# MVME-HBUT/Faster-OreFSDet

Measured on AMD Instinct MI355X. Metric: images/sec at 640x640 25-shot (eval FPS: model(inputs) + device sync per image, bs=1 per GPU), higher is better.
Workload: dtype f32

## Files before the change

faster-orefsdet_amd/csrc/ore_common.h:

```cpp
#pragma once
#include <hip/hip_runtime.h>
#include <stdint.h>
#include <stdio.h>
#include "ore_hip.h"

void ore_set_error(const char* fmt, ...);
void ore_note_wino(int v);
int ore_last_wino(void);
void ore_note_launch(int code, int split);
void ore_flop_count_add(double flops);

#define ORE_CHECK_ARG(cond, ...)              \
    do {                                      \
        if (!(cond)) {                        \
            ore_set_error(__VA_ARGS__);       \
            return ORE_EINVAL;                \
        }                                     \
    } while (0)

#define ORE_HIP(call)                                                                   \
    do {                                                                                \
        hipError_t e_ = (call);                                                         \
        if (e_ != hipSuccess) {                                                         \
            ore_set_error("%s:%d %s -> %s", __FILE__, __LINE__, #call, hipGetErrorString(e_)); \
// ... 26 lines not shown
}

typedef __bf16 bf16x8_t __attribute__((ext_vector_type(8)));
__device__ __forceinline__ f32x4 from_bf16x4(s16x4 h) {
    const u32x2 u = __builtin_bit_cast(u32x2, h);
    return f32x4{__builtin_bit_cast(float, u.x << 16), __builtin_bit_cast(float, u.x & 0xffff0000u),
                 __builtin_bit_cast(float, u.y << 16), __builtin_bit_cast(float, u.y & 0xffff0000u)};
}
__device__ __forceinline__ float bf16_bits_to_f32(unsigned short h) { return __builtin_bit_cast(float, (unsigned)h << 16); }
struct ore_bf16_t { unsigned short v; };
__device__ __forceinline__ f32x4 ld4(const float* p) { return *reinterpret_cast<const f32x4*>(p); }
__device__ __forceinline__ f32x4 ld4(const ore_bf16_t* p) { return from_bf16x4(*reinterpret_cast<const s16x4*>(p)); }
__device__ __forceinline__ void st4(float* p, f32x4 v) { *reinterpret_cast<f32x4*>(p) = v; }
__device__ __forceinline__ void st4(ore_bf16_t* p, f32x4 v) { *reinterpret_cast<s16x4*>(p) = to_bf16x4(v); }
__device__ __forceinline__ float ld1(const float* p) { return *p; }
__device__ __forceinline__ float ld1(const ore_bf16_t* p) { return bf16_bits_to_f32(p->v); }

namespace oreroi {
int roi_predict_post(const float* h, int32_t C, int32_t h_parts, const float* h_bias, const float* cls_w, const float* cls_b,
                     const float* box_w, const float* box_b, const float* boxes, const int32_t* n_dev, int32_t n_host, int32_t cap,
                     const float* reg_weights4_host, float img_h, float img_w, float score_thresh, float nms_thresh,
                     int32_t topk, float* det_boxes, float* det_scores, int64_t* det_src, int32_t* det_count,
                     const float* post_dev, float* fin_boxes, float* fin_scores, int32_t* fin_count,
                     int32_t* host_count, void* workspace, size_t workspace_bytes, void* stream);
int roi_merge_classes(const float* det_boxes, const float* det_scores, const int32_t* det_count, int32_t K, int32_t cap,
                      const int64_t* class_ids, int32_t topk, const float* post_dev, float* fin_boxes, float* fin_scores,
                      int64_t* fin_classes, int32_t* fin_count, int32_t* host_count, void* stream);
struct PredictWs { size_t raw_boxes, c_boxes, raw_scores, c_scores, c_src, ok, keep, nms; };
inline PredictWs predict_ws_layout(int32_t cap) {
    const size_t c = (size_t)(cap > 0 ? cap : 1);
    PredictWs w{};
    size_t o = 256;
    w.raw_boxes = o; o += c * 16;
    w.c_boxes = o; o += c * 16;
    w.raw_scores = o; o += c * 4;
    w.c_scores = o; o += c * 4;
    w.c_src = o; o += c * 4;
    w.ok = o; o += c * 4;
    w.keep = o; o += c * 8;
    w.nms = (o + 255) & ~(size_t)255;
    return w;
}
}

namespace oremisc {
int correlation_classes(const float* q, int32_t q_ld, int32_t q_coff, int32_t n_levels, const int32_t* H, const int32_t* W, int32_t C,
                        int32_t K, const float* k11s, const float* k13s, const float* k31s, float* out, int32_t out_ld, void* stream);
// ... 3 lines not shown
```

faster-orefsdet_amd/csrc/ore_conv_internal.h:

```cpp
#pragma once
#include "ore_common.h"

namespace oreconv {

struct Lvl { int orow0, irow0, H, W, Ho, Wo; };

struct ConvP {
    const float* in; int in_ld, in_coff;
    int B, Cin;
    int nlev; Lvl lv[4];
    const float* w;
    int Cout, Cout16, kh, kw, stride, pad, M, K;
    const float* scale; const float* shift; int ep_stride; int relu_cout;
    const float* in_mul; const float* in_add; int in_relu;
    const float* add; int add_ld, add_coff, add_H, add_W;
    float* out; int out_ld, out_coff;
    float* colsum;
    int splitk, steps_per_split, nchunks;
    float* ws; int* tile_cnt;
    int bf16;
    int xmap;
    int sb;
    const float* wino;
    size_t w_lstride;
// ... 49 lines not shown
    X(64, 112, 4, 1) X(64, 128, 2, 2) X(64, 64, 2, 2) X(128, 64, 4, 1) X(128, 128, 2, 2) X(32, 128, 1, 4) X(128, 112, 4, 1) X(64, 80, 4, 1) X(32, 64, 2, 2)
#define ORE_KW_TILES(X) \
    X(16, 16) X(16, 32) X(16, 48) X(16, 64) X(16, 80) X(32, 16) X(32, 32) X(32, 48) X(32, 64) X(32, 80)
constexpr bool gs_fits(int bm, int bn, int ns) { return ((bm + bn) / 16 + 3) / 4 * (ns - 1) <= 63 && (size_t)ns * (bm + bn) * 64 <= 150 * 1024; }

struct ConvKnobs {
    int patch_mode = -1;
    int kw_mode = 1;
    int kw_force[4] = {};
    int gs_force[2] = {};
    int gs_ns = 3;
    int xmap_force = -1;
    int kw_nw_force = 0;
    int wino_mode = 1;
    int ws_sb_mode = 1;
    int ws_s2_mode = 1;
    int rf_mode = 1;
    int rf_force[3] = {};
    int kd_mode = 1;
    int kd_force[4] = {};
    int gd_mode = 1;
    int gd_force[3] = {};
    int gd_dbg = 0;
    int igemm[5] = {};
};
extern ConvKnobs g_knobs;

using ConvPlan = ore_conv_plan_t;
ConvPlan conv_plan(const ConvP& p, int req_splitk, size_t workspace_floats);
bool conv_wino_covers(int Cout, int Cin);
int wino_level_blocks(const ConvP& p, int gy, int* blk0);

int launch_ws(const ConvP& p, const ConvPlan& pl, hipStream_t st);
int launch_patch(const ConvP& p, const ConvPlan& pl, hipStream_t st);
int launch_igemm(const ConvP& p, const ConvPlan& pl, hipStream_t st);
int launch_wino(const ConvP& p, const ConvPlan& pl, hipStream_t st);
int launch_gd(const ConvP& p, const ConvPlan& pl, hipStream_t st);
int launch_kd(const ConvP& p, const ConvPlan& pl, hipStream_t st);
int launch_rf(const ConvP& p, const ConvPlan& pl, hipStream_t st);
int launch_gs(const ConvP& p, const ConvPlan& pl, hipStream_t st);
int launch_kw(const ConvP& p, const ConvPlan& pl, hipStream_t st);
int conv_gd_splitk(const float* in, int in_ld, const float* w, int M, int K, int Cout16, float* parts, int S, hipStream_t st);

}
```

faster-orefsdet_amd/csrc/ore_conv_plan.cpp:

```cpp
#include "ore_common.h"
#include "ore_conv_internal.h"

namespace oreconv {

ConvKnobs g_knobs;

namespace {

const ConvKnobs& K = g_knobs;

ConvPlan make_plan(int launcher, int bm, int bn, int b0, int b1, int b2, int b3, int gx, int gy, int xmap = 0, int splitk = 1, int sps = 0) {
    ConvPlan pl{};
    pl.launcher = launcher; pl.error = ORE_OK;
    pl.bm = bm; pl.bn = bn;
    pl.build[0] = b0; pl.build[1] = b1; pl.build[2] = b2; pl.build[3] = b3;
    pl.splitk = splitk; pl.steps_per_split = sps; pl.xmap = xmap;
    pl.gx = gx; pl.gy = gy;
    return pl;
}

ConvPlan none() { return ConvPlan{}; }

ConvPlan fail(int code) {
    ConvPlan pl{};
// ... 487 lines not shown
}

using namespace oreconv;

extern "C" int ore_conv_set_plan_override(int32_t BM, int32_t BN, int32_t WGM, int32_t WGN, int32_t WGK) {
    ConvKnobs& k = g_knobs;
    switch (BM) {
    case -1: k.patch_mode = BN; k.igemm[0] = 0; break;
    case -2: k.kw_mode = BN; k.igemm[0] = 0; break;
    case -3: k.kw_force[0] = BN; k.kw_force[1] = WGM; k.kw_force[2] = WGN; k.kw_force[3] = WGK; break;
    case -4: k.gs_force[0] = BN; k.gs_force[1] = WGM; if (WGN > 0) k.gs_ns = WGN; break;
    case -5: k.xmap_force = BN; break;
    case -6: k.kw_nw_force = BN; break;
    case -7: k.wino_mode = BN; break;
    case -8: k.ws_sb_mode = BN; break;
    case -9: k.ws_s2_mode = BN; break;
    case -10: k.rf_mode = BN; break;
    case -11: k.rf_force[0] = BN; k.rf_force[1] = WGM; k.rf_force[2] = WGN; break;
    case -12: k.kd_mode = BN; break;
    case -13: k.kd_force[0] = BN; k.kd_force[1] = WGM; k.kd_force[2] = WGN; k.kd_force[3] = WGK; break;
    case -14: k.gd_mode = BN; break;
    case -15: k.gd_force[0] = BN; k.gd_force[1] = WGM; k.gd_force[2] = WGN; break;
    case -16: k.gd_dbg = BN; break;
    default: k.igemm[0] = BM; k.igemm[1] = BN; k.igemm[2] = WGM; k.igemm[3] = WGN; k.igemm[4] = WGK; break;
    }
    return ORE_OK;
}

extern "C" int ore_conv_reset_plan_overrides(void) {
    g_knobs = ConvKnobs{};
    return ORE_OK;
}
```

faster-orefsdet_amd/csrc/ore_engine.hip:

```cpp
#include <map>
#include <string>
#include <vector>
#include <math.h>
#include <string.h>
#include "ore_common.h"
#include "ore_conv_internal.h"
#include <algorithm>


namespace {

struct HostTensor { std::vector<float> v; std::vector<int64_t> shape; };

struct Conv {
    float* w = nullptr; float* scale = nullptr; float* shift = nullptr;
    uint16_t* wh = nullptr;
    float* wino = nullptr;
    int Cin = 0, Cout = 0, k = 1, stride = 1, pad = 0, relu_cout = 0;
};

struct Buf { float* p = nullptr; int ld = 0; size_t rows = 0; };

struct Geo { int B, H, W, Hp, Wp; int h[6], w[6]; };

// ... 417 lines not shown
int run_detect_classes(ore_engine* e, const Geo& g, hipStream_t st, int K) {
    ore_detect_desc d[ORE_MAX_CLASSES];
    for (int k = 0; k < K; ++k) {
        d[k] = ore_detect_desc{};
        detect_desc(e, g, k, d[k]);
        if (k > 0) d[k].workspace = e->det_ws_slots + (size_t)(k - 1) * e->det_ws_bytes;
    }
    return ore_detect_batch_fwd(d, K, st);
}

int run_roi(ore_engine* e, const Geo& g, hipStream_t st, double* flops, int b = 0, bool class_slot = false) {
    const ore_model_cfg& c = e->cfg;
    float* roi_W = class_slot ? e->roi_W_slot[b] : e->roi_W;
    float* roi_b = class_slot ? e->roi_b_slot[b] : e->roi_b;
    const int F = c.fpn_ch;
    const size_t cap = (size_t)3 * c.pre_topk, rcap = (size_t)e->roi_cap;
    float* out_boxes = e->out_boxes + b * cap * 4;
    int32_t* counts = e->counts + b * 4;
    const float* feat[3]; int ld[3], coff[3], H[3], W[3]; float sc[3];
    for (int l = 0; l < 3; ++l) {
        feat[l] = e->at(e->pcat.p, ((size_t)lvl_row0(g, l) + (size_t)b * g.h[l + 3] * g.w[l + 3]) * 2 * F); ld[l] = 2 * F; coff[l] = F;
        H[l] = g.h[l + 3]; W[l] = g.w[l + 3]; sc[l] = 1.0f / (float)c.strides[l];
    }
    int rc = e->sb() ? ore_roi_align_bf16_fwd(reinterpret_cast<const uint16_t* const*>(feat), ld, coff, H, W, sc, 3, 3, F, e->roi_pooled, out_boxes,
                                              counts + 1, 0, e->roi_cap, e->roi_feat, st)
                     : ore_roi_align_fwd(feat, ld, coff, H, W, sc, 3, 3, F, e->roi_pooled, out_boxes, counts + 1, 0, e->roi_cap, e->roi_feat, st);
    if (rc) return rc;
    const int K = e->roi_pooled * e->roi_pooled * F;
    Run r{e, st};
    r.prof = e->profiling;
    Conv fc{};
    fc.w = roi_W; fc.scale = nullptr; fc.shift = roi_b; fc.Cin = K; fc.Cout = e->roi_fc; fc.k = 1; fc.stride = 1; fc.pad = 0;
    fc.relu_cout = e->roi_fc;
    const int S = e->roi_ksplit;
    if (S > 1) {
        const double fl = 2.0 * (double)e->roi_cap * K * e->roi_fc;
        hipEvent_t ea = nullptr, eb = nullptr;
        size_t ia = 0;
        if (r.prof) { ia = e->ev_used; ea = e->next_event(); eb = e->next_event(); if (ea) (void)hipEventRecord(ea, st); }
        rc = oreconv::conv_gd_splitk(e->roi_feat, K, roi_W, e->roi_cap, K, e->roi_fc, e->roi_hp, S, st);
        if (r.prof && ea && eb) { (void)hipEventRecord(eb, st); e->spans.push_back({ia, ia + 1, fl, fl}); }
        if (rc) return rc;
        *flops = fl;
    } else {
        PrecisionScope fp32(ORE_CONV_FP32);
        r.conv(fc, e->roi_feat, K, 0, 1, 1, e->roi_cap, e->roi_h, e->roi_fc, 0);
        if (r.rc) return r.rc;
        *flops = r.flops;
    }
    return oreroi::roi_predict_post(S > 1 ? e->roi_hp : e->roi_h, e->roi_fc, S > 1 ? S : 0, S > 1 ? roi_b : nullptr, e->roi_cls_w, e->roi_cls_b,
                                    e->roi_box_w, e->roi_box_b, out_boxes, counts + 1, 0,
                                    e->roi_cap, e->roi_reg_w, (float)g.H, (float)g.W, e->roi_score_thresh, e->roi_nms_thresh, e->roi_topk,
                                    e->det_boxes + b * rcap * 4, e->det_scores + b * rcap, e->det_src + b * rcap, e->det_count + b * 4,
                                    class_slot ? nullptr : e->post, e->fin_boxes_of(b), e->fin_scores_of(b), e->fin_count + b * 4,
                                    b == 0 && !class_slot ? e->pin_count_dev : nullptr, e->roi_ws, e->roi_ws_bytes, st);
}

}

extern "C" int ore_engine_set_roi_head(ore_engine* e, const float* W_host, const float* b_host, int32_t fc_dim, int32_t pooled,
                                       const float* cls_w_host, const float* cls_b_host, const float* box_w_host,
                                       const float* box_b_host, const float* reg_weights4_host, float score_thresh, float nms_thresh,
                                       int32_t topk) {
    ORE_CHECK_ARG(e && e->finalized && W_host && b_host && cls_w_host && cls_b_host && box_w_host && box_b_host && reg_weights4_host,
                  "ore_engine_set_roi_head: engine must be finalized, pointers non-null");
    ORE_CHECK_ARG(fc_dim % 16 == 0 && fc_dim > 0 && pooled >= 1 && pooled <= 16 && nms_thresh > 0.f, "ore_engine_set_roi_head: bad args");
    ORE_CHECK_ARG((size_t)fc_dim * 4 * 71 + 6 * 64 * 4 <= 60 * 1024,
                  "ore_engine_set_roi_head: fc width %d: the fused second-stage kernels cover fc widths up to 208 (FC_DIM/8 = 128 in finetune_vovnet.yaml)", fc_dim);
    static_assert(ORE_DET_RECORD_ROWS <= 512, "k_roi_tail<1024> sorts at most 512 candidates");
    ORE_HIP(hipSetDevice(e->device));
    const size_t K = (size_t)pooled * pooled * e->cfg.fpn_ch;
    int rc;
    auto up = [&](float** dst, const float* src, size_t n) -> int {
        if (!*dst && (rc = e->dalloc(dst, n))) return rc;
        ORE_HIP(hipMemcpy(*dst, src, n * sizeof(float), hipMemcpyHostToDevice));
        return ORE_OK;
    };
    if (e->roi_set && (e->roi_fc != fc_dim || e->roi_pooled != pooled)) { ore_set_error("ore_engine_set_roi_head: shape change not supported"); return ORE_EINVAL; }
// ... 629 lines not shown
```

faster-orefsdet_amd/csrc/ore_roi.hip:

```cpp
#include "ore_common.h"
#include <stdlib.h>

#ifdef ORE_TRACE
__device__ unsigned long long* g_trace_roi = nullptr;
#define ROI_TR(i) do { if (g_trace_roi && threadIdx.x == 0) g_trace_roi[(i)] = __builtin_amdgcn_s_memtime(); } while (0)
extern "C" int ore_debug_set_trace_roi(unsigned long long* buf) {
    return hipMemcpyToSymbol(HIP_SYMBOL(g_trace_roi), &buf, sizeof(buf)) == hipSuccess ? 0 : -5;
}
#else
#define ROI_TR(i) do { } while (0)
#endif

namespace {

__device__ __forceinline__ float ore_expf(float x) {
    if (x > 88.0f) x = 88.0f;
    if (x < -87.0f) x = -87.0f;
    const float n = rintf(x * 1.44269504088896341f);
    float r = fmaf(n, -0.693359375f, x);
    r = fmaf(n, 2.12194440e-4f, r);
    float p = 1.9875691500e-4f;
    p = fmaf(p, r, 1.3981999507e-3f);
    p = fmaf(p, r, 8.3334519073e-3f);
    p = fmaf(p, r, 4.1665795894e-2f);
    p = fmaf(p, r, 1.6666665459e-1f);
    p = fmaf(p, r, 5.0000001201e-1f);
    const float e = fmaf(p, r * r, r) + 1.0f;
    const int ni = (int)n;
    return e * __uint_as_float((unsigned)(ni + 127) << 23);
}

struct RoiP {
    const void* feat[4]; int ld[4], coff[4], H[4], W[4]; float scale[4];
    int n_levels, min_level, C, pooled;
    float canonical_size; int canonical_level;
    const float* boxes; const int* n_ptr; int n_host; int cap;
    float* out;
    const int* bidx;
};

template <typename TS>
__device__ __forceinline__ f32x4 bilinear4(const TS* f, int ld, int H, int W, float y, float x, int c) {
    if (y < -1.0f || y > (float)H || x < -1.0f || x > (float)W) return f32x4{0.f, 0.f, 0.f, 0.f};
    if (y <= 0.f) y = 0.f;
    if (x <= 0.f) x = 0.f;
    int y_low = (int)y, x_low = (int)x, y_high, x_high;
    if (y_low >= H - 1) { y_high = y_low = H - 1; y = (float)y_low; } else y_high = y_low + 1;
    if (x_low >= W - 1) { x_high = x_low = W - 1; x = (float)x_low; } else x_high = x_low + 1;
    const float ly = y - (float)y_low, lx = x - (float)x_low, hy = 1.f - ly, hx = 1.f - lx;
    const f32x4 v1 = ld4(f + (size_t)(y_low * W + x_low) * ld + c);
    const f32x4 v2 = ld4(f + (size_t)(y_low * W + x_high) * ld + c);
    const f32x4 v3 = ld4(f + (size_t)(y_high * W + x_low) * ld + c);
    const f32x4 v4 = ld4(f + (size_t)(y_high * W + x_high) * ld + c);
    return (hy * hx) * v1 + (hy * lx) * v2 + (ly * hx) * v3 + (ly * lx) * v4;
}

constexpr int ROI_FWD_SPLIT = 8;
template <typename TS>
__global__ __launch_bounds__(256) void k_roi_align(RoiP p) {
    const int r = blockIdx.x / ROI_FWD_SPLIT, part = blockIdx.x % ROI_FWD_SPLIT;
    const int n = min(p.n_ptr ? *p.n_ptr : p.n_host, p.cap);
    const int P = p.pooled, C4 = p.C >> 2;
    float* dst = p.out + (size_t)r * P * P * p.C;
    if (r >= n) {
        for (int i = part * 256 + threadIdx.x; i < P * P * C4; i += 256 * ROI_FWD_SPLIT) *reinterpret_cast<f32x4*>(dst + i * 4) = f32x4{0.f, 0.f, 0.f, 0.f};
        return;
    }
    const f32x4 b = *reinterpret_cast<const f32x4*>(p.boxes + (size_t)r * 4);
    const float size = sqrtf((b.z - b.x) * (b.w - b.y));
    float lv = floorf((float)p.canonical_level + log2f(size / p.canonical_size + 1e-8f));
    lv = fminf(fmaxf(lv, (float)p.min_level), (float)(p.min_level + p.n_levels - 1));
    const int l = (int)lv - p.min_level;
    const float sc = p.scale[l];
    const int H = p.H[l], W = p.W[l], ld = p.ld[l];
    const TS* f = reinterpret_cast<const TS*>(p.feat[l]) + p.coff[l] + (p.bidx ? (size_t)p.bidx[r] * H * W * ld : 0);
    const float x0 = b.x * sc - 0.5f, y0 = b.y * sc - 0.5f, x1 = b.z * sc - 0.5f, y1 = b.w * sc - 0.5f;
    const float rw = x1 - x0, rh = y1 - y0;
    const float bw = rw / (float)P, bh = rh / (float)P;
    const int gh = (int)ceilf(rh / (float)P), gw = (int)ceilf(rw / (float)P);
    const float cnt = (float)max(gh * gw, 1);
    for (int i = part * 256 + threadIdx.x; i < P * P * C4; i += 256 * ROI_FWD_SPLIT) {
        const int c = (i % C4) * 4, bin = i / C4;
// ... 524 lines not shown
    }
    if (tid == 0) *p.c_count = base_sh;
}

__global__ __launch_bounds__(256) void k_roi_finalize(const long long* __restrict__ keep, const int* __restrict__ n_keep, int topk,
                                                      const float* __restrict__ c_boxes, const float* __restrict__ c_scores,
                                                      const int* __restrict__ c_src, float* __restrict__ det_boxes,
                                                      float* __restrict__ det_scores, long long* __restrict__ det_src,
                                                      int* __restrict__ det_count) {
    int n = *n_keep;
    if (topk >= 0 && n > topk) n = topk;
    for (int i = threadIdx.x; i < n; i += 256) {
        const long long k = keep[i];
        *reinterpret_cast<f32x4*>(det_boxes + (size_t)i * 4) = *reinterpret_cast<const f32x4*>(c_boxes + (size_t)k * 4);
        det_scores[i] = c_scores[k];
        det_src[i] = (long long)c_src[k];
    }
    if (threadIdx.x == 0) *det_count = n;
}


constexpr int ROI_FUSED_CAP = 512;

template <int RPB>
__global__ __launch_bounds__(256) void k_roi_predict_mb(PredP p, int* __restrict__ ok_out) {
    extern __shared__ float hs[];
    const int C = p.C, LDH = C + 1;
    float* dots = hs + RPB * LDH;
    const int tid = threadIdx.x, lane = tid & 63, wave = __builtin_amdgcn_readfirstlane(tid >> 6);
    const int r0 = blockIdx.x * RPB;
    if (p.h_parts > 0) {
        const size_t zs = (size_t)p.cap * C;
        const int ne = max(min(RPB, p.cap - r0), 0) * C;
        for (int i0 = tid; i0 < ne; i0 += 256 * 4) {
            float v[4];
            const float* src[4];
#pragma unroll
            for (int j = 0; j < 4; ++j) {
                const int i = min(i0 + 256 * j, ne - 1);
                v[j] = p.h_bias ? p.h_bias[i % C] : 0.0f;
                src[j] = p.h + (size_t)r0 * C + i;
            }
            for (int z0 = 0; z0 < p.h_parts; z0 += 16) {
                float t[16][4];
#pragma unroll
                for (int k = 0; k < 16; ++k)
#pragma unroll
                    for (int j = 0; j < 4; ++j) t[k][j] = z0 + k < p.h_parts ? src[j][(size_t)(z0 + k) * zs] : 0.0f;
#pragma unroll
                for (int k = 0; k < 16; ++k)
#pragma unroll
                    for (int j = 0; j < 4; ++j) v[j] += t[k][j];
            }
#pragma unroll
            for (int j = 0; j < 4; ++j) {
                const int i = i0 + 256 * j;
                if (i < ne) hs[(i / C) * LDH + (i % C)] = fmaxf(v[j], 0.0f);
            }
        }
    }
    const int n = min(p.n_ptr ? *p.n_ptr : p.n_host, p.cap);
    if (r0 >= n) {
        if (tid < RPB && r0 + tid < p.cap) ok_out[r0 + tid] = 0;
        return;
    }
    const int rows = min(RPB, n - r0);
    if (p.h_parts <= 0) {
        for (int i = tid; i < rows * C; i += 256) hs[(i / C) * LDH + (i % C)] = p.h[(size_t)r0 * C + i];
    }
    __syncthreads();
    if (wave < 3 && lane < rows) {
        const float* h = hs + lane * LDH;
        const float* __restrict__ w0 = wave == 0 ? p.cls_w : p.box_w + (size_t)(2 * wave - 2) * C;
        const float* __restrict__ w1 = w0 + C;
        float a0 = wave == 0 ? p.cls_b[0] : p.box_b[2 * wave - 2];
        float a1 = wave == 0 ? p.cls_b[1] : p.box_b[2 * wave - 1];
#pragma unroll 8
        for (int c = 0; c < C; ++c) {
            const float v = h[c];
            a0 = fmaf(w0[c], v, a0);
            a1 = fmaf(w1[c], v, a1);
        }
        dots[(2 * wave) * 64 + lane] = a0;
        dots[(2 * wave + 1) * 64 + lane] = a1;
    }
    __syncthreads();
    if (wave == 0 && lane < RPB && r0 + lane < p.cap) {
        const int r = r0 + lane;
        int ok = 0;
        if (lane < rows) {
            const float l0 = dots[lane], l1 = dots[64 + lane];
            const float d0 = dots[128 + lane], d1 = dots[192 + lane], d2 = dots[256 + lane], d3 = dots[320 + lane];
            const float m = fmaxf(l0, l1);
            const float e0 = ore_expf(l0 - m), e1 = ore_expf(l1 - m);
            const float score = e0 / (e0 + e1);
            const f32x4 b = *reinterpret_cast<const f32x4*>(p.boxes + (size_t)r * 4);
            const float w = b.z - b.x, hgt = b.w - b.y;
            const float cx = b.x + 0.5f * w, cy = b.y + 0.5f * hgt;
            const float dx = d0 / p.wx, dy = d1 / p.wy;
            const float dw = fminf(d2 / p.ww, p.scale_clamp), dh = fminf(d3 / p.wh, p.scale_clamp);
            const float pcx = dx * w + cx, pcy = dy * hgt + cy;
            const float pw = ore_expf(dw) * w, phh = ore_expf(dh) * hgt;
            f32x4 ob = f32x4{pcx - 0.5f * pw, pcy - 0.5f * phh, pcx + 0.5f * pw, pcy + 0.5f * phh};
            const bool finite = isfinite(ob.x) && isfinite(ob.y) && isfinite(ob.z) && isfinite(ob.w) && isfinite(score);
            ob.x = fminf(fmaxf(ob.x, 0.f), p.img_w); ob.y = fminf(fmaxf(ob.y, 0.f), p.img_h);
            ob.z = fminf(fmaxf(ob.z, 0.f), p.img_w); ob.w = fminf(fmaxf(ob.w, 0.f), p.img_h);
            *reinterpret_cast<f32x4*>(p.raw_boxes + (size_t)r * 4) = ob;
            p.raw_scores[r] = score;
            ok = (finite && score > p.score_thresh) ? 1 : 0;
        }
        ok_out[r] = ok;
    }
}

struct TailP {
    const float* raw_boxes; const float* raw_scores; const int* ok; const int* n_ptr; int n_host; int cap;
    float nms_thresh; int topk;
    float* det_boxes; float* det_scores; long long* det_src; int* det_count;
    const float* post;
    float* fin_boxes; float* fin_scores; int* fin_count; int* host_count;
};

__device__ __forceinline__ unsigned long long wave_or64(unsigned long long v) {
#pragma unroll
    for (int d = 32; d > 0; d >>= 1) {
        const unsigned lo = __shfl_xor((unsigned)v, d), hi = __shfl_xor((unsigned)(v >> 32), d);
        v |= ((unsigned long long)hi << 32) | lo;
    }
    return v;
}

template <int T>
__global__ __launch_bounds__(T) void k_roi_tail(TailP p) {
    unsigned long long rec_early = 0ull;
    if (p.post != nullptr && p.host_count)
        rec_early = __hip_atomic_load(reinterpret_cast<unsigned long long*>(p.host_count) + 1, __ATOMIC_RELAXED, __HIP_MEMORY_SCOPE_SYSTEM);
    __shared__ __attribute__((aligned(16))) float cb[ROI_FUSED_CAP * 4];
    __shared__ float cs[ROI_FUSED_CAP];
    __shared__ int csrc[ROI_FUSED_CAP];
    __shared__ __attribute__((aligned(16))) float sb[ROI_FUSED_CAP * 4];
    __shared__ float sa[ROI_FUSED_CAP];
    __shared__ int sord[ROI_FUSED_CAP];
    __shared__ unsigned long long supT[ROI_FUSED_CAP * (ROI_FUSED_CAP / 64)];
    __shared__ int wsum[T / 64];
    __shared__ int keep_pos[ROI_FUSED_CAP];
    __shared__ int sh_keep, sh_stop;
    constexpr int NW = T / 64, WPR = ROI_FUSED_CAP / 64;
    const int tid = threadIdx.x, lane = tid & 63, wave = tid >> 6;
    int ok_first = 0;
    f32x4 box_first = {0.f, 0.f, 0.f, 0.f};
    float score_first = 0.f;
    if (tid < p.cap) {
        ok_first = p.ok[tid];
        box_first = *reinterpret_cast<const f32x4*>(p.raw_boxes + (size_t)tid * 4);
        score_first = p.raw_scores[tid];
    }
    ROI_TR(0);
    const int n = min(p.n_ptr ? *p.n_ptr : p.n_host, p.cap);
    ROI_TR(1);
    int base = 0;
    for (int r0 = 0; r0 < n; r0 += T) {
        const int r = r0 + tid;
        const int ok = (r < n) ? (r0 == 0 ? ok_first : p.ok[r]) : 0;
        int inc = ok;
#pragma unroll
        for (int d = 1; d < 64; d <<= 1) { const int t = __shfl_up(inc, d); if (lane >= d) inc += t; }
        if (lane == 63) wsum[wave] = inc;
        __syncthreads();
        int pre = base, tot = 0;
// ... 140 lines not shown
            __syncthreads();
            int pre = fbase, tot = 0;
            for (int w2 = 0; w2 < NW; ++w2) { const int s2 = wsum[w2]; if (w2 < wave) pre += s2; tot += s2; }
            if (ok) {
                const int pos = pre + inc - 1;
                *reinterpret_cast<f32x4*>(p.fin_boxes + (size_t)pos * 4) = b;
                p.fin_scores[pos] = sc;
                if (rec) {
                    *reinterpret_cast<f32x4*>(rec_boxes + (size_t)pos * 4) = b;
                    rec_scores[pos] = sc;
                    rec_cls[pos] = 0ll;
                }
            }
            fbase += tot;
        }
        if (tid == 0) {
            *p.fin_count = fbase;
            if (p.host_count) *p.host_count = fbase;
        }
        ROI_TR(7);
    }
}

constexpr int MERGE_MAX_CLASSES = 16;
constexpr int MERGE_MAX_ROWS = MERGE_MAX_CLASSES * ROI_FUSED_CAP;

struct MergeP {
    const float* det_boxes; const float* det_scores; const int* det_count; int K, cap; const long long* class_ids; int topk;
    const float* post; float* fin_boxes; float* fin_scores; long long* fin_classes; int* fin_count; int* host_count;
};

template <int T>
__global__ __launch_bounds__(T) void k_roi_merge_classes(MergeP p) {
    unsigned long long rec_early = 0ull;
    if (p.host_count)
        rec_early = __hip_atomic_load(reinterpret_cast<unsigned long long*>(p.host_count) + 1, __ATOMIC_RELAXED, __HIP_MEMORY_SCOPE_SYSTEM);
    __shared__ float sc[MERGE_MAX_ROWS];
    __shared__ __attribute__((aligned(16))) float sel_b[ROI_FUSED_CAP * 4];
    __shared__ float sel_s[ROI_FUSED_CAP];
    __shared__ int sel_k[ROI_FUSED_CAP];
    __shared__ int off[MERGE_MAX_CLASSES + 1];
    __shared__ int wsum[T / 64];
    constexpr int NW = T / 64;
    const int tid = threadIdx.x, lane = tid & 63, wave = tid >> 6;
    if (tid == 0) {
        int o = 0;
// ... 67 lines not shown
                rec_cls[pos] = cls;
            }
        }
        fbase += tot;
    }
    __syncthreads();
    if (tid == 0) {
        *p.fin_count = fbase;
        if (p.host_count) {
            __threadfence_system();
            *p.host_count = fbase;
        }
    }
}

}

extern "C" int ore_nms_device_n_fwd(const float* boxes, const float* scores, const int32_t* n_dev, int32_t cap, float thr,
                                    int64_t* keep_idx, int32_t* count, void* workspace, size_t workspace_bytes, void* stream);

static int roi_align_fwd_impl(const void* const* feat, const int32_t* ld, const int32_t* coff, const int32_t* H, const int32_t* W,
                              const float* scales_host, int32_t n_levels, int32_t min_level, int32_t C, int32_t pooled,
                              const float* boxes, const int32_t* n_dev, int32_t n_host, int32_t cap, float* out, void* stream,
                              const int32_t* box_image, int feat_bf16);

extern "C" int ore_roi_align_fwd(const float* const* feat, const int32_t* ld, const int32_t* coff, const int32_t* H, const int32_t* W,
                                 const float* scales_host, int32_t n_levels, int32_t min_level, int32_t C, int32_t pooled,
                                 const float* boxes, const int32_t* n_dev, int32_t n_host, int32_t cap, float* out, void* stream) {
    return roi_align_fwd_impl((const void* const*)feat, ld, coff, H, W, scales_host, n_levels, min_level, C, pooled, boxes, n_dev, n_host, cap, out, stream, nullptr, 0);
}

extern "C" int ore_roi_align_batched_fwd(const float* const* feat, const int32_t* ld, const int32_t* coff, const int32_t* H, const int32_t* W,
                                         const float* scales_host, int32_t n_levels, int32_t min_level, int32_t C, int32_t pooled,
                                         const float* boxes, const int32_t* box_image, int32_t n, float* out, void* stream) {
    ORE_CHECK_ARG(box_image, "ore_roi_align_batched_fwd: null box_image");
    return roi_align_fwd_impl((const void* const*)feat, ld, coff, H, W, scales_host, n_levels, min_level, C, pooled, boxes, nullptr, n, n, out, stream, box_image, 0);
}

static int roi_align_fwd_impl(const void* const* feat, const int32_t* ld, const int32_t* coff, const int32_t* H, const int32_t* W,
                              const float* scales_host, int32_t n_levels, int32_t min_level, int32_t C, int32_t pooled,
                              const float* boxes, const int32_t* n_dev, int32_t n_host, int32_t cap, float* out, void* stream,
                              const int32_t* box_image, int feat_bf16) {
    ORE_CHECK_ARG(feat && ld && coff && H && W && scales_host && boxes && out, "ore_roi_align_fwd: null pointer");
    ORE_CHECK_ARG(n_levels >= 1 && n_levels <= 4 && C % 4 == 0 && pooled >= 1 && pooled <= 16 && cap >= 1, "ore_roi_align_fwd: bad args");
    RoiP p{};
    for (int l = 0; l < n_levels; ++l) {
        ORE_CHECK_ARG(feat[l] && ld[l] % 4 == 0 && coff[l] % 4 == 0 && H[l] > 0 && W[l] > 0, "ore_roi_align_fwd: level %d", l);
        p.feat[l] = feat[l]; p.ld[l] = ld[l]; p.coff[l] = coff[l]; p.H[l] = H[l]; p.W[l] = W[l]; p.scale[l] = scales_host[l];
    }
    p.n_levels = n_levels; p.min_level = min_level; p.C = C; p.pooled = pooled;
    p.canonical_size = 224.0f; p.canonical_level = 4;
    p.boxes = boxes; p.n_ptr = n_dev; p.n_host = n_host; p.cap = cap; p.out = out; p.bidx = box_image;
    if (feat_bf16) hipLaunchKernelGGL(k_roi_align<ore_bf16_t>, dim3(cap * ROI_FWD_SPLIT), dim3(256), 0, (hipStream_t)stream, p);
    else hipLaunchKernelGGL(k_roi_align<float>, dim3(cap * ROI_FWD_SPLIT), dim3(256), 0, (hipStream_t)stream, p);
    return ore_launch_status("k_roi_align");
}

extern "C" int ore_roi_align_bf16_fwd(const uint16_t* const* feat, const int32_t* ld, const int32_t* coff, const int32_t* H, const int32_t* W,
                                      const float* scales_host, int32_t n_levels, int32_t min_level, int32_t C, int32_t pooled,
                                      const float* boxes, const int32_t* n_dev, int32_t n_host, int32_t cap, float* out, void* stream) {
    return roi_align_fwd_impl((const void* const*)feat, ld, coff, H, W, scales_host, n_levels, min_level, C, pooled, boxes, n_dev, n_host, cap, out,
                              stream, nullptr, 1);
}

extern "C" size_t ore_roi_predict_workspace_bytes(int32_t cap) {
    const size_t c = (size_t)(cap > 0 ? cap : 1);
    return 256 + c * 16 * 2 + c * 4 * 4 + c * 8 + ore_nms_workspace_bytes(cap) + 4096;
}

extern "C" int ore_roi_predict_fwd(const float* h, int32_t C, const float* cls_w, const float* cls_b, const float* box_w,
                                   const float* box_b, const float* boxes, const int32_t* n_dev, int32_t n_host, int32_t cap,
                                   const float* reg_weights4_host, float img_h, float img_w, float score_thresh, float nms_thresh,
                                   int32_t topk, float* det_boxes, float* det_scores, int64_t* det_src, int32_t* det_count,
                                   void* workspace, size_t workspace_bytes, void* stream) {
    return ore_roi_predict_post_fwd(h, C, cls_w, cls_b, box_w, box_b, boxes, n_dev, n_host, cap, reg_weights4_host, img_h, img_w,
                                    score_thresh, nms_thresh, topk, det_boxes, det_scores, det_src, det_count, nullptr, nullptr, nullptr,
                                    nullptr, nullptr, workspace, workspace_bytes, stream);
}

extern "C" int ore_roi_predict_post_fwd(const float* h, int32_t C, const float* cls_w, const float* cls_b, const float* box_w,
                                        const float* box_b, const float* boxes, const int32_t* n_dev, int32_t n_host, int32_t cap,
                                        const float* reg_weights4_host, float img_h, float img_w, float score_thresh, float nms_thresh,
                                        int32_t topk, float* det_boxes, float* det_scores, int64_t* det_src, int32_t* det_count,
                                        const float* post_dev, float* fin_boxes, float* fin_scores, int32_t* fin_count,
                                        int32_t* host_count, void* workspace, size_t workspace_bytes, void* stream) {
    return oreroi::roi_predict_post(h, C, 0, nullptr, cls_w, cls_b, box_w, box_b, boxes, n_dev, n_host, cap, reg_weights4_host, img_h, img_w,
                                    score_thresh, nms_thresh, topk, det_boxes, det_scores, det_src, det_count, post_dev, fin_boxes, fin_scores,
                                    fin_count, host_count, workspace, workspace_bytes, stream);
}

int oreroi::roi_predict_post(const float* h, int32_t C, int32_t h_parts, const float* h_bias, const float* cls_w, const float* cls_b,
                             const float* box_w, const float* box_b, const float* boxes, const int32_t* n_dev, int32_t n_host, int32_t cap,
                             const float* reg_weights4_host, float img_h, float img_w, float score_thresh, float nms_thresh,
                             int32_t topk, float* det_boxes, float* det_scores, int64_t* det_src, int32_t* det_count,
                             const float* post_dev, float* fin_boxes, float* fin_scores, int32_t* fin_count,
                             int32_t* host_count, void* workspace, size_t workspace_bytes, void* stream) {
    ORE_CHECK_ARG(h && cls_w && cls_b && box_w && box_b && boxes && reg_weights4_host && det_boxes && det_scores && det_src && det_count &&
                      workspace, "ore_roi_predict_fwd: null pointer");
    ORE_CHECK_ARG(cap >= 1 && C >= 1, "ore_roi_predict_fwd: bad args");
    ORE_CHECK_ARG(!post_dev || (fin_boxes && fin_scores && fin_count), "ore_roi_predict_post_fwd: post without outputs");
    ORE_CHECK_ARG(!post_dev || cap <= ROI_FUSED_CAP, "ore_roi_predict_post_fwd: the fused postprocess covers cap <= %d", ROI_FUSED_CAP);
    if (workspace_bytes < ore_roi_predict_workspace_bytes(cap)) {
        ore_set_error("ore_roi_predict_fwd: workspace %zu < %zu", workspace_bytes, ore_roi_predict_workspace_bytes(cap));
        return ORE_ENOMEM;
    }
    char* ws = (char*)workspace;
    const oreroi::PredictWs L = oreroi::predict_ws_layout(cap);
    int* c_count = (int*)ws; int* n_keep = c_count + 1;
    float* raw_boxes = (float*)(ws + L.raw_boxes);
    float* c_boxes = (float*)(ws + L.c_boxes);
    float* raw_scores = (float*)(ws + L.raw_scores);
    float* c_scores = (float*)(ws + L.c_scores);
    int* c_src = (int*)(ws + L.c_src);
    int* ok = (int*)(ws + L.ok);
    long long* keep = (long long*)(ws + L.keep);
    const size_t o = L.nms;
    void* nms_ws = ws + o;
    PredP p{};
    p.h = h; p.C = C; p.h_parts = h_parts; p.h_bias = h_bias; p.cls_w = cls_w; p.cls_b = cls_b; p.box_w = box_w; p.box_b = box_b;
    p.boxes = boxes; p.n_ptr = n_dev; p.n_host = n_host; p.cap = cap;
    p.wx = reg_weights4_host[0]; p.wy = reg_weights4_host[1]; p.ww = reg_weights4_host[2]; p.wh = reg_weights4_host[3];
    p.scale_clamp = logf(1000.0f / 16.0f);
    p.img_h = img_h; p.img_w = img_w; p.score_thresh = score_thresh;
    p.raw_boxes = raw_boxes; p.raw_scores = raw_scores; p.c_boxes = c_boxes; p.c_scores = c_scores; p.c_src = c_src; p.c_count = c_count;
    hipStream_t st = (hipStream_t)stream;
    if (cap <= ROI_FUSED_CAP && (size_t)C * 4 * 71 + 6 * 64 * 4 <= 60 * 1024) {
        const size_t lds = ((size_t)64 * (C + 1) + 6 * 64) * sizeof(float);
        if (h_parts > 0) hipLaunchKernelGGL(k_roi_predict_mb<8>, dim3(ceil_div(cap, 8)), dim3(256), lds, st, p, ok);
        else hipLaunchKernelGGL(k_roi_predict_mb<64>, dim3(ceil_div(cap, 64)), dim3(256), lds, st, p, ok);
        int rc = ore_launch_status("k_roi_predict_mb");
        if (rc) return rc;
        TailP t{};
        t.raw_boxes = raw_boxes; t.raw_scores = raw_scores; t.ok = ok; t.n_ptr = n_dev; t.n_host = n_host; t.cap = cap;
        t.nms_thresh = nms_thresh; t.topk = topk;
        t.det_boxes = det_boxes; t.det_scores = det_scores; t.det_src = (long long*)det_src; t.det_count = det_count;
        t.post = post_dev; t.fin_boxes = fin_boxes; t.fin_scores = fin_scores; t.fin_count = fin_count;
        t.host_count = host_count;
        hipLaunchKernelGGL(k_roi_tail<1024>, dim3(1), dim3(1024), 0, st, t);
        return ore_launch_status("k_roi_tail");
    }
    ORE_CHECK_ARG(h_parts == 0, "roi_predict_post: K-split partial sums are summed by the fused path only (cap <= %d)", ROI_FUSED_CAP);
    ORE_CHECK_ARG(!post_dev, "ore_roi_predict_post_fwd: the fused postprocess covers fc width <= %d (got %d) and cap <= %d (got %d)",
                  (int)((60 * 1024 - 6 * 64 * 4) / (4 * 71)), C, ROI_FUSED_CAP, cap);
    const size_t lds = ((size_t)256 * (C + 1) + 6 * (size_t)C) * sizeof(float);
    ORE_CHECK_ARG(lds <= 150 * 1024, "ore_roi_predict_fwd: fc width %d too large", C);
    if (lds > 48 * 1024) ORE_HIP(hipFuncSetAttribute((const void*)k_roi_predict, hipFuncAttributeMaxDynamicSharedMemorySize, (int)lds));
    hipLaunchKernelGGL(k_roi_predict, dim3(1), dim3(256), lds, st, p);
    int rc = ore_launch_status("k_roi_predict");
    if (rc) return rc;
    rc = ore_nms_device_n_fwd(c_boxes, c_scores, c_count, cap, nms_thresh, (int64_t*)keep, n_keep, nms_ws,
                              workspace_bytes - o, st);
    if (rc) return rc;
    hipLaunchKernelGGL(k_roi_finalize, dim3(1), dim3(256), 0, st, keep, n_keep, topk, c_boxes, c_scores, c_src, det_boxes, det_scores,
                       (long long*)det_src, det_count);
    return ore_launch_status("k_roi_finalize");
}

static int roi_align_bwd_impl(float* const* dfeat, const int32_t* ld, const int32_t* coff, const int32_t* H, const int32_t* W,
                              const float* scales_host, int32_t n_levels, int32_t min_level, int32_t C, int32_t pooled,
                              const float* boxes, const int32_t* box_image, int32_t n, const float* dout, long long* const* acc,
// ... 100 lines not shown
```

Baseline: 1652.

## Fuse ROI predict and NMS tail via last-block ticket

Merges the per-row ROI predict kernel and the single-block NMS/finalize tail into one launch. The last block to finish, found through an atomic ticket counter, runs the tail and reuses the tail's LDS struct as staging for the predict rows. ROI align zeroes the ticket word, so no separate memset is needed. This removes one kernel launch and its gap per image. In exchange, every block now uses 1024 threads and the large tail LDS footprint, which lowers occupancy for the predict phase, and correctness depends on acquire/release fences.

```diff
diff --git a/faster-orefsdet_amd/csrc/ore_common.h b/faster-orefsdet_amd/csrc/ore_common.h
--- a/faster-orefsdet_amd/csrc/ore_common.h
+++ b/faster-orefsdet_amd/csrc/ore_common.h
@@ -72,7 +72,11 @@
                      const float* reg_weights4_host, float img_h, float img_w, float score_thresh, float nms_thresh,
                      int32_t topk, float* det_boxes, float* det_scores, int64_t* det_src, int32_t* det_count,
                      const float* post_dev, float* fin_boxes, float* fin_scores, int32_t* fin_count,
-                     int32_t* host_count, void* workspace, size_t workspace_bytes, void* stream);
+                     int32_t* host_count, void* workspace, size_t workspace_bytes, void* stream, bool ticket_zeroed = false);
+inline int32_t* roi_predict_ticket(void* workspace) { return reinterpret_cast<int32_t*>(workspace) + 2; }
+int roi_align_fwd(const void* const* feat, const int32_t* ld, const int32_t* coff, const int32_t* H, const int32_t* W,
+                  const float* scales_host, int32_t n_levels, int32_t min_level, int32_t C, int32_t pooled, const float* boxes,
+                  const int32_t* n_dev, int32_t cap, float* out, int feat_bf16, int32_t* zero_word, void* stream);
 int roi_merge_classes(const float* det_boxes, const float* det_scores, const int32_t* det_count, int32_t K, int32_t cap,
                       const int64_t* class_ids, int32_t topk, const float* post_dev, float* fin_boxes, float* fin_scores,
                       int64_t* fin_classes, int32_t* fin_count, int32_t* host_count, void* stream);
diff --git a/faster-orefsdet_amd/csrc/ore_conv_internal.h b/faster-orefsdet_amd/csrc/ore_conv_internal.h
--- a/faster-orefsdet_amd/csrc/ore_conv_internal.h
+++ b/faster-orefsdet_amd/csrc/ore_conv_internal.h
@@ -95,6 +95,7 @@
     int gd_mode = 1;
     int gd_force[3] = {};
     int gd_dbg = 0;
+    int roi_tail_fused = 1;
     int igemm[5] = {};
 };
 extern ConvKnobs g_knobs;
diff --git a/faster-orefsdet_amd/csrc/ore_conv_plan.cpp b/faster-orefsdet_amd/csrc/ore_conv_plan.cpp
--- a/faster-orefsdet_amd/csrc/ore_conv_plan.cpp
+++ b/faster-orefsdet_amd/csrc/ore_conv_plan.cpp
@@ -533,6 +533,7 @@
     case -14: k.gd_mode = BN; break;
     case -15: k.gd_force[0] = BN; k.gd_force[1] = WGM; k.gd_force[2] = WGN; break;
     case -16: k.gd_dbg = BN; break;
+    case -17: k.roi_tail_fused = BN; break;
     default: k.igemm[0] = BM; k.igemm[1] = BN; k.igemm[2] = WGM; k.igemm[3] = WGN; k.igemm[4] = WGK; break;
     }
     return ORE_OK;
diff --git a/faster-orefsdet_amd/csrc/ore_engine.hip b/faster-orefsdet_amd/csrc/ore_engine.hip
--- a/faster-orefsdet_amd/csrc/ore_engine.hip
+++ b/faster-orefsdet_amd/csrc/ore_engine.hip
@@ -463,9 +463,8 @@
         feat[l] = e->at(e->pcat.p, ((size_t)lvl_row0(g, l) + (size_t)b * g.h[l + 3] * g.w[l + 3]) * 2 * F); ld[l] = 2 * F; coff[l] = F;
         H[l] = g.h[l + 3]; W[l] = g.w[l + 3]; sc[l] = 1.0f / (float)c.strides[l];
     }
-    int rc = e->sb() ? ore_roi_align_bf16_fwd(reinterpret_cast<const uint16_t* const*>(feat), ld, coff, H, W, sc, 3, 3, F, e->roi_pooled, out_boxes,
-                                              counts + 1, 0, e->roi_cap, e->roi_feat, st)
-                     : ore_roi_align_fwd(feat, ld, coff, H, W, sc, 3, 3, F, e->roi_pooled, out_boxes, counts + 1, 0, e->roi_cap, e->roi_feat, st);
+    int rc = oreroi::roi_align_fwd(reinterpret_cast<const void* const*>(feat), ld, coff, H, W, sc, 3, 3, F, e->roi_pooled, out_boxes, counts + 1,
+                                   e->roi_cap, e->roi_feat, e->sb() ? 1 : 0, oreroi::roi_predict_ticket(e->roi_ws), st);
     if (rc) return rc;
     const int K = e->roi_pooled * e->roi_pooled * F;
     Run r{e, st};
@@ -494,7 +493,7 @@
                                     e->roi_cap, e->roi_reg_w, (float)g.H, (float)g.W, e->roi_score_thresh, e->roi_nms_thresh, e->roi_topk,
                                     e->det_boxes + b * rcap * 4, e->det_scores + b * rcap, e->det_src + b * rcap, e->det_count + b * 4,
                                     class_slot ? nullptr : e->post, e->fin_boxes_of(b), e->fin_scores_of(b), e->fin_count + b * 4,
-                                    b == 0 && !class_slot ? e->pin_count_dev : nullptr, e->roi_ws, e->roi_ws_bytes, st);
+                                    b == 0 && !class_slot ? e->pin_count_dev : nullptr, e->roi_ws, e->roi_ws_bytes, st, true);
 }
 
 }
diff --git a/faster-orefsdet_amd/csrc/ore_roi.hip b/faster-orefsdet_amd/csrc/ore_roi.hip
--- a/faster-orefsdet_amd/csrc/ore_roi.hip
+++ b/faster-orefsdet_amd/csrc/ore_roi.hip
@@ -1,4 +1,4 @@
-#include "ore_common.h"
+#include "ore_conv_internal.h"
 #include <stdlib.h>
 
 #ifdef ORE_TRACE
@@ -37,6 +37,7 @@
     const float* boxes; const int* n_ptr; int n_host; int cap;
     float* out;
     const int* bidx;
+    int* zero_word;
 };
 
 template <typename TS>
@@ -58,6 +59,7 @@
 constexpr int ROI_FWD_SPLIT = 8;
 template <typename TS>
 __global__ __launch_bounds__(256) void k_roi_align(RoiP p) {
+    if (p.zero_word && blockIdx.x == 0 && threadIdx.x == 0) *p.zero_word = 0;
     const int r = blockIdx.x / ROI_FWD_SPLIT, part = blockIdx.x % ROI_FWD_SPLIT;
     const int n = min(p.n_ptr ? *p.n_ptr : p.n_host, p.cap);
     const int P = p.pooled, C4 = p.C >> 2;
@@ -628,39 +630,39 @@
 
 constexpr int ROI_FUSED_CAP = 512;
 
-template <int RPB>
-__global__ __launch_bounds__(256) void k_roi_predict_mb(PredP p, int* __restrict__ ok_out) {
-    extern __shared__ float hs[];
+template <int RPB, int NT>
+__device__ __forceinline__ void roi_predict_rows(const PredP& p, int* __restrict__ ok_out, float* hs) {
     const int C = p.C, LDH = C + 1;
     float* dots = hs + RPB * LDH;
     const int tid = threadIdx.x, lane = tid & 63, wave = __builtin_amdgcn_readfirstlane(tid >> 6);
     const int r0 = blockIdx.x * RPB;
     if (p.h_parts > 0) {
+        constexpr int EPT = 1024 / NT;
         const size_t zs = (size_t)p.cap * C;
         const int ne = max(min(RPB, p.cap - r0), 0) * C;
-        for (int i0 = tid; i0 < ne; i0 += 256 * 4) {
-            float v[4];
-            const float* src[4];
-#pragma unroll
-            for (int j = 0; j < 4; ++j) {
-                const int i = min(i0 + 256 * j, ne - 1);
+        for (int i0 = tid; i0 < ne; i0 += NT * EPT) {
+            float v[EPT];
+            const float* src[EPT];
+#pragma unroll
+            for (int j = 0; j < EPT; ++j) {
+                const int i = min(i0 + NT * j, ne - 1);
                 v[j] = p.h_bias ? p.h_bias[i % C] : 0.0f;
                 src[j] = p.h + (size_t)r0 * C + i;
             }
             for (int z0 = 0; z0 < p.h_parts; z0 += 16) {
-                float t[16][4];
+                float t[16][EPT];
 #pragma unroll
                 for (int k = 0; k < 16; ++k)
 #pragma unroll
-                    for (int j = 0; j < 4; ++j) t[k][j] = z0 + k < p.h_parts ? src[j][(size_t)(z0 + k) * zs] : 0.0f;
+                    for (int j = 0; j < EPT; ++j) t[k][j] = z0 + k < p.h_parts ? src[j][(size_t)(z0 + k) * zs] : 0.0f;
 #pragma unroll
                 for (int k = 0; k < 16; ++k)
 #pragma unroll
-                    for (int j = 0; j < 4; ++j) v[j] += t[k][j];
-            }
-#pragma unroll
-            for (int j = 0; j < 4; ++j) {
-                const int i = i0 + 256 * j;
+                    for (int j = 0; j < EPT; ++j) v[j] += t[k][j];
+            }
+#pragma unroll
+            for (int j = 0; j < EPT; ++j) {
+                const int i = i0 + NT * j;
                 if (i < ne) hs[(i / C) * LDH + (i % C)] = fmaxf(v[j], 0.0f);
             }
         }
@@ -672,7 +674,7 @@
     }
     const int rows = min(RPB, n - r0);
     if (p.h_parts <= 0) {
-        for (int i = tid; i < rows * C; i += 256) hs[(i / C) * LDH + (i % C)] = p.h[(size_t)r0 * C + i];
+        for (int i = tid; i < rows * C; i += NT) hs[(i / C) * LDH + (i % C)] = p.h[(size_t)r0 * C + i];
     }
     __syncthreads();
     if (wave < 3 && lane < rows) {
@@ -719,6 +721,12 @@
     }
 }
 
+template <int RPB>
+__global__ __launch_bounds__(256) void k_roi_predict_mb(PredP p, int* __restrict__ ok_out) {
+    extern __shared__ float hs[];
+    roi_predict_rows<RPB, 256>(p, ok_out, hs);
+}
+
 struct TailP {
     const float* raw_boxes; const float* raw_scores; const int* ok; const int* n_ptr; int n_host; int cap;
     float nms_thresh; int topk;
@@ -737,20 +745,28 @@
 }
 
 template <int T>
-__global__ __launch_bounds__(T) void k_roi_tail(TailP p) {
+struct TailLds {
+    alignas(16) float cb[ROI_FUSED_CAP * 4];
+    float cs[ROI_FUSED_CAP];
+    int csrc[ROI_FUSED_CAP];
+    alignas(16) float sb[ROI_FUSED_CAP * 4];
+    float sa[ROI_FUSED_CAP];
+    int sord[ROI_FUSED_CAP];
+    unsigned long long supT[ROI_FUSED_CAP * (ROI_FUSED_CAP / 64)];
+    int wsum[T / 64];
+    int keep_pos[ROI_FUSED_CAP];
+    int sh_keep, sh_stop, sh_last;
+};
+constexpr size_t ROI_TAIL_STAGE_FLOATS = sizeof(unsigned long long) * ROI_FUSED_CAP * (ROI_FUSED_CAP / 64) / sizeof(float);
+
+template <int T>
+__device__ __forceinline__ void roi_tail_run(const TailP& p, TailLds<T>& L) {
     unsigned long long rec_early = 0ull;
     if (p.post != nullptr && p.host_count)
         rec_early = __hip_atomic_load(reinterpret_cast<unsigned long long*>(p.host_count) + 1, __ATOMIC_RELAXED, __HIP_MEMORY_SCOPE_SYSTEM);
-    __shared__ __attribute__((aligned(16))) float cb[ROI_FUSED_CAP * 4];
-    __shared__ float cs[ROI_FUSED_CAP];
-    __shared__ int csrc[ROI_FUSED_CAP];
-    __shared__ __attribute__((aligned(16))) float sb[ROI_FUSED_CAP * 4];
-    __shared__ float sa[ROI_FUSED_CAP];
-    __shared__ int sord[ROI_FUSED_CAP];
-    __shared__ unsigned long long supT[ROI_FUSED_CAP * (ROI_FUSED_CAP / 64)];
-    __shared__ int wsum[T / 64];
-    __shared__ int keep_pos[ROI_FUSED_CAP];
-    __shared__ int sh_keep, sh_stop;
+    float* cb = L.cb; float* cs = L.cs; int* csrc = L.csrc; float* sb = L.sb; float* sa = L.sa; int* sord = L.sord;
+    unsigned long long* supT = L.supT; int* wsum = L.wsum; int* keep_pos = L.keep_pos;
+    int& sh_keep = L.sh_keep; int& sh_stop = L.sh_stop;
     constexpr int NW = T / 64, WPR = ROI_FUSED_CAP / 64;
     const int tid = threadIdx.x, lane = tid & 63, wave = tid >> 6;
     int ok_first = 0;
@@ -937,6 +953,33 @@
     }
 }
 
+template <int T>
+__global__ __launch_bounds__(T) void k_roi_tail(TailP p) {
+    __shared__ TailLds<T> L;
+    roi_tail_run<T>(p, L);
+}
+
+template <int RPB, int T>
+__global__ __launch_bounds__(T) void k_roi_predict_tail(PredP p, int* __restrict__ ok_out, TailP t, int* __restrict__ ticket) {
+    __shared__ TailLds<T> L;
+    roi_predict_rows<RPB, T>(p, ok_out, reinterpret_cast<float*>(L.supT));
+    asm volatile("s_waitcnt vmcnt(0)" ::: "memory");
+    __syncthreads();
+    if (threadIdx.x == 0) {
+        __builtin_amdgcn_fence(__ATOMIC_RELEASE, "agent");
+        asm volatile("s_waitcnt vmcnt(0)" ::: "memory");
+        const int last = __hip_atomic_fetch_add(ticket, 1, __ATOMIC_RELAXED, __HIP_MEMORY_SCOPE_AGENT) == (int)gridDim.x - 1;
+        if (last) {
+            __builtin_amdgcn_fence(__ATOMIC_ACQUIRE, "agent");
+            asm volatile("s_waitcnt vmcnt(0)" ::: "memory");
+        }
+        L.sh_last = last;
+    }
+    __syncthreads();
+    if (!L.sh_last) return;
+    roi_tail_run<T>(t, L);
+}
+
 constexpr int MERGE_MAX_CLASSES = 16;
 constexpr int MERGE_MAX_ROWS = MERGE_MAX_CLASSES * ROI_FUSED_CAP;
 
@@ -1050,7 +1093,7 @@
 static int roi_align_fwd_impl(const void* const* feat, const int32_t* ld, const int32_t* coff, const int32_t* H, const int32_t* W,
                               const float* scales_host, int32_t n_levels, int32_t min_level, int32_t C, int32_t pooled,
                               const float* boxes, const int32_t* n_dev, int32_t n_host, int32_t cap, float* out, void* stream,
-                              const int32_t* box_image, int feat_bf16);
+                              const int32_t* box_image, int feat_bf16, int32_t* zero_word = nullptr);
 
 extern "C" int ore_roi_align_fwd(const float* const* feat, const int32_t* ld, const int32_t* coff, const int32_t* H, const int32_t* W,
                                  const float* scales_host, int32_t n_levels, int32_t min_level, int32_t C, int32_t pooled,
@@ -1068,7 +1111,7 @@
 static int roi_align_fwd_impl(const void* const* feat, const int32_t* ld, const int32_t* coff, const int32_t* H, const int32_t* W,
                               const float* scales_host, int32_t n_levels, int32_t min_level, int32_t C, int32_t pooled,
                               const float* boxes, const int32_t* n_dev, int32_t n_host, int32_t cap, float* out, void* stream,
-                              const int32_t* box_image, int feat_bf16) {
+                              const int32_t* box_image, int feat_bf16, int32_t* zero_word) {
     ORE_CHECK_ARG(feat && ld && coff && H && W && scales_host && boxes && out, "ore_roi_align_fwd: null pointer");
     ORE_CHECK_ARG(n_levels >= 1 && n_levels <= 4 && C % 4 == 0 && pooled >= 1 && pooled <= 16 && cap >= 1, "ore_roi_align_fwd: bad args");
     RoiP p{};
@@ -1079,6 +1122,7 @@
     p.n_levels = n_levels; p.min_level = min_level; p.C = C; p.pooled = pooled;
     p.canonical_size = 224.0f; p.canonical_level = 4;
     p.boxes = boxes; p.n_ptr = n_dev; p.n_host = n_host; p.cap = cap; p.out = out; p.bidx = box_image;
+    p.zero_word = zero_word;
     if (feat_bf16) hipLaunchKernelGGL(k_roi_align<ore_bf16_t>, dim3(cap * ROI_FWD_SPLIT), dim3(256), 0, (hipStream_t)stream, p);
     else hipLaunchKernelGGL(k_roi_align<float>, dim3(cap * ROI_FWD_SPLIT), dim3(256), 0, (hipStream_t)stream, p);
     return ore_launch_status("k_roi_align");
@@ -1089,6 +1133,13 @@
                                       const float* boxes, const int32_t* n_dev, int32_t n_host, int32_t cap, float* out, void* stream) {
     return roi_align_fwd_impl((const void* const*)feat, ld, coff, H, W, scales_host, n_levels, min_level, C, pooled, boxes, n_dev, n_host, cap, out,
                               stream, nullptr, 1);
+}
+
+int oreroi::roi_align_fwd(const void* const* feat, const int32_t* ld, const int32_t* coff, const int32_t* H, const int32_t* W,
+                          const float* scales_host, int32_t n_levels, int32_t min_level, int32_t C, int32_t pooled, const float* boxes,
+                          const int32_t* n_dev, int32_t cap, float* out, int feat_bf16, int32_t* zero_word, void* stream) {
+    return roi_align_fwd_impl(feat, ld, coff, H, W, scales_host, n_levels, min_level, C, pooled, boxes, n_dev, 0, cap, out, stream, nullptr,
+                              feat_bf16, zero_word);
 }
 
 extern "C" size_t ore_roi_predict_workspace_bytes(int32_t cap) {
@@ -1122,7 +1173,7 @@
                              const float* reg_weights4_host, float img_h, float img_w, float score_thresh, float nms_thresh,
                              int32_t topk, float* det_boxes, float* det_scores, int64_t* det_src, int32_t* det_count,
                              const float* post_dev, float* fin_boxes, float* fin_scores, int32_t* fin_count,
-                             int32_t* host_count, void* workspace, size_t workspace_bytes, void* stream) {
+                             int32_t* host_count, void* workspace, size_t workspace_bytes, void* stream, bool ticket_zeroed) {
     ORE_CHECK_ARG(h && cls_w && cls_b && box_w && box_b && boxes && reg_weights4_host && det_boxes && det_scores && det_src && det_count &&
                       workspace, "ore_roi_predict_fwd: null pointer");
     ORE_CHECK_ARG(cap >= 1 && C >= 1, "ore_roi_predict_fwd: bad args");
@@ -1153,17 +1204,23 @@
     p.raw_boxes = raw_boxes; p.raw_scores = raw_scores; p.c_boxes = c_boxes; p.c_scores = c_scores; p.c_src = c_src; p.c_count = c_count;
     hipStream_t st = (hipStream_t)stream;
     if (cap <= ROI_FUSED_CAP && (size_t)C * 4 * 71 + 6 * 64 * 4 <= 60 * 1024) {
-        const size_t lds = ((size_t)64 * (C + 1) + 6 * 64) * sizeof(float);
-        if (h_parts > 0) hipLaunchKernelGGL(k_roi_predict_mb<8>, dim3(ceil_div(cap, 8)), dim3(256), lds, st, p, ok);
-        else hipLaunchKernelGGL(k_roi_predict_mb<64>, dim3(ceil_div(cap, 64)), dim3(256), lds, st, p, ok);
-        int rc = ore_launch_status("k_roi_predict_mb");
-        if (rc) return rc;
         TailP t{};
         t.raw_boxes = raw_boxes; t.raw_scores = raw_scores; t.ok = ok; t.n_ptr = n_dev; t.n_host = n_host; t.cap = cap;
         t.nms_thresh = nms_thresh; t.topk = topk;
         t.det_boxes = det_boxes; t.det_scores = det_scores; t.det_src = (long long*)det_src; t.det_count = det_count;
         t.post = post_dev; t.fin_boxes = fin_boxes; t.fin_scores = fin_scores; t.fin_count = fin_count;
         t.host_count = host_count;
+        if (h_parts > 0 && oreconv::g_knobs.roi_tail_fused && (size_t)8 * (C + 1) + 6 * 64 <= ROI_TAIL_STAGE_FLOATS) {
+            int32_t* ticket = oreroi::roi_predict_ticket(workspace);
+            if (!ticket_zeroed) ORE_HIP(hipMemsetAsync(ticket, 0, sizeof(int32_t), st));
+            hipLaunchKernelGGL((k_roi_predict_tail<8, 1024>), dim3(ceil_div(cap, 8)), dim3(1024), 0, st, p, ok, t, ticket);
+            return ore_launch_status("k_roi_predict_tail");
+        }
+        const size_t lds = ((size_t)64 * (C + 1) + 6 * 64) * sizeof(float);
+        if (h_parts > 0) hipLaunchKernelGGL(k_roi_predict_mb<8>, dim3(ceil_div(cap, 8)), dim3(256), lds, st, p, ok);
+        else hipLaunchKernelGGL(k_roi_predict_mb<64>, dim3(ceil_div(cap, 64)), dim3(256), lds, st, p, ok);
+        int rc = ore_launch_status("k_roi_predict_mb");
+        if (rc) return rc;
         hipLaunchKernelGGL(k_roi_tail<1024>, dim3(1), dim3(1024), 0, st, t);
         return ore_launch_status("k_roi_tail");
     }
```

Result: no change. 1648 (median of 3 runs) (-0.3%).
